# oxidecomputer/ingot

Measured on AMD Instinct MI355X. Metric: Mpkt/s device-resident L2/L3/L4 parse, 64–1500 B frames; % HBM roofline, higher is better.
Workload: dtype u8; 1 GPU; C2: 1,048,576 x 64 B Eth/IPv4/UDP per GPU, 64-B slots, UdpParser; frames_per_gpu=1048576, frames_total=1048576, chain=UdpParser, record_bytes=16, streams=2, arena_copies_rotated=8, record_buffers_rotated=8, timing_mode=launches

## Files before the change

### ingot_amd/csrc/ring.hip

```cpp
#include "walk.h"

namespace ingot_gpu {
namespace {

template <uint32_t NCH, uint32_t DEPTH, int CHAIN, int MODE, uint32_t POL = 0>
__global__ __launch_bounds__(BLOCK) void k_parse_pipe(ParseArgs a) {
    constexpr uint32_t WIN = NCH * 16u;
    const uint32_t pol = POL ? POL : a.policy;
    constexpr uint32_t WAVE_DW = WAVE * NCH * 4u;
    constexpr uint32_t IMG_DW = WAVES * WAVE_DW + 16u;
    __shared__ __attribute__((aligned(16))) uint32_t s_img[DEPTH * IMG_DW];
    const uint32_t lane = threadIdx.x & (WAVE - 1u);
    const uint32_t wave = threadIdx.x / WAVE;
    uint32_t* img0 = s_img + wave * WAVE_DW;
    const uint64_t ntiles = (a.n + WAVE - 1u) / WAVE;
    const uint32_t take = a.stride < WIN ? a.stride : WIN;

    auto stage = [&](uint64_t tt, uint32_t* img) {
#pragma unroll
        for (uint32_t k = 0; k < NCH; ++k) {
            const uint32_t q = k * WAVE + lane;
            const uint32_t pp = q / NCH;
            const uint32_t c = (q - pp * NCH) ^ swz<NCH>(pp);
            uint64_t slot = tt * WAVE + pp;
            if (slot >= a.n) slot = a.n - 1u;
            stage16p(a.arena + slot * a.stride + 16u * c, img + k * WAVE * 4u, pol);
        }
    };
    auto parse = [&](uint64_t tt, const uint32_t* img) {
        const uint64_t i = tt * WAVE + lane;
        Frame<NCH> fr{(const lds_u32*)img, lane, 0u, take, a.stride, a.arena + i * a.stride};
        Rec r;
        walk<CHAIN, false>(fr, r, nullptr, nullptr);
        if (i < a.n) {
            if constexpr (MODE == OUT_REC8) store_rec(static_cast<uint2*>(a.out) + i, pack8(r), pol);
            else store_rec(static_cast<uint4*>(a.out) + i, pack(r), pol);
        }
    };

    uint32_t bid = blockIdx.x;
    if ((a.xcd_remap & 1u) && gridDim.x % 8u == 0u)
        bid = (bid % 8u) * (gridDim.x / 8u) + bid / 8u;
    const uint64_t gw = (uint64_t)bid * WAVES + wave;
    const uint64_t nw = (uint64_t)gridDim.x * WAVES;
    uint64_t t, step, tend;
    if ((a.xcd_remap & 4u) && gridDim.x % 8u == 0u) {
        const uint64_t x = blockIdx.x % 8u;
        const uint64_t nwx = (uint64_t)(gridDim.x / 8u) * WAVES;
        const uint64_t region = (ntiles + 7u) / 8u;
        t = x * region + (uint64_t)(blockIdx.x / 8u) * WAVES + wave;
        tend = (x + 1u) * region < ntiles ? (x + 1u) * region : ntiles;
        step = nwx;
    } else if (a.xcd_remap & 2u) {
        const uint64_t J = (ntiles + nw - 1u) / nw;
        t = gw * J;
        tend = t + J < ntiles ? t + J : ntiles;
        step = 1u;
    } else {
        t = gw;
        tend = ntiles;
        step = nw;
    }
    if (t >= tend) return;
    if constexpr (DEPTH == 1) {
        stage(t, img0);
        asm volatile("s_waitcnt vmcnt(0)" ::: "memory");
        for (;;) {
            const uint64_t i = t * WAVE + lane;
            Frame<NCH> fr{(const lds_u32*)img0, lane, 0u, take, a.stride, a.arena + i * a.stride};
            Rec r;
            walk<CHAIN, false>(fr, r, nullptr, nullptr);
            asm volatile("s_waitcnt lgkmcnt(0)" ::: "memory");
            const uint64_t tn = t + step;
            const bool more = tn < tend;
            if (more) stage(tn, img0);
            if (i < a.n) {
                if constexpr (MODE == OUT_REC8) store_rec(static_cast<uint2*>(a.out) + i, pack8(r), pol);
                else store_rec(static_cast<uint4*>(a.out) + i, pack(r), pol);
            }
            if (!more) break;
            t = tn;
            asm volatile("s_waitcnt vmcnt(1)" ::: "memory");
        }
        return;
    }
#pragma unroll
    for (uint32_t d = 0; d + 1u < DEPTH; ++d)
        if (t + d * step < tend) stage(t + d * step, img0 + d * IMG_DW);
    for (uint32_t j = 0;; ++j) {
        const uint64_t tn = t + (DEPTH - 1u) * step;
        if (tn < tend) {
            stage(tn, img0 + ((j + DEPTH - 1u) % DEPTH) * IMG_DW);
            if (j + 1u >= DEPTH)
                asm volatile("s_waitcnt vmcnt(%0)" ::"n"((DEPTH - 1u) * (NCH + 1u)) : "memory");
            else
                asm volatile("s_waitcnt vmcnt(%0)" ::"n"((DEPTH - 1u) * NCH) : "memory");
        } else {
            asm volatile("s_waitcnt vmcnt(0)" ::: "memory");
        }
        parse(t, img0 + (j % DEPTH) * IMG_DW);
        t += step;
        if (t >= tend) break;
    }
}

__device__ __forceinline__ uint32_t load_system_u32(const uint32_t* p) {
    uint32_t v;
    asm volatile("global_load_dword %0, %1, off sc0 sc1\n\ts_waitcnt vmcnt(0)"
                 : "=v"(v)
                 : "v"(p)
                 : "memory");
    return (uint32_t)__builtin_amdgcn_readfirstlane((int)v);
}

template <uint32_t NCH, uint32_t DEPTH, int CHAIN, int MODE>
__global__ __launch_bounds__(BLOCK) void k_parse_ring(RingArgs a) {
    constexpr uint32_t WIN = NCH * 16u;
    constexpr uint32_t WAVE_DW = WAVE * NCH * 4u;
    constexpr uint32_t IMG_DW = WAVES * WAVE_DW + 16u;
    __shared__ __attribute__((aligned(16))) uint32_t s_img[DEPTH * IMG_DW];
    const uint32_t lane = threadIdx.x & (WAVE - 1u);
    const uint32_t wave = (uint32_t)__builtin_amdgcn_readfirstlane((int)(threadIdx.x / WAVE));
    uint32_t* img0 = s_img + wave * WAVE_DW;
    const uint32_t tpb = a.tiles_per_batch;
    const uint32_t G = a.groups;
    const uint32_t grp = (blockIdx.x / 8u) % G;
    const uint32_t gblk = (blockIdx.x / (8u * G)) * 8u + blockIdx.x % 8u;
    const uint32_t W = (gridDim.x / G) * WAVES;
    const uint32_t nbg = (a.nbatches - grp + G - 1u) / G;
    const uint32_t total = tpb * nbg;
    const uint32_t g0 = gblk * WAVES + wave;
    if (g0 >= total) return;
    const uint32_t J = (total - g0 + W - 1u) / W;
    uint64_t n = a.n;
    uint32_t stride = a.stride, policy = a.policy, nb = a.nbatches;
    asm volatile("" : "+s"(n), "+s"(stride), "+s"(policy), "+s"(nb));
    const uint32_t take = stride < WIN ? stride : WIN;
    uint32_t avail = a.published;
    bool live = true;

    auto ready = [&](uint32_t b) -> bool {
        if (b < avail) return true;
        if (!a.doorbell) return false;
        const uint64_t t0 = wall_clock64();
        uint32_t naps = 1;
        for (;;) {
            const uint32_t v = load_system_u32(a.doorbell);
            if (v >= a.db_first + b) {
                const uint32_t pub = v - a.db_first + 1u;
                avail = pub < a.nbatches ? pub : a.nbatches;
                __builtin_amdgcn_fence(__ATOMIC_ACQUIRE, "");
                return true;
            }
            if (wall_clock64() - t0 > a.timeout_ticks) {
                if (a.status && lane == 0) atomicOr(a.status, 1u);
                return false;
            }
            for (uint32_t z = 0; z < naps; ++z) __builtin_amdgcn_s_sleep(32);
            naps = naps < 8u ? 2u * naps : 8u;
        }
    };
    struct Cur {
        uint32_t b, t;
        const uint8_t* arena;
        void* out;
    };
    auto setb = [&](Cur& c) {
        if (c.b < nb) {
            c.arena = a.b[c.b].arena;
            c.out = a.b[c.b].out;
            asm volatile("" : "+s"(c.arena), "+s"(c.out));
        }
    };
    auto adv = [&](Cur& c) {
        c.t += W;
        if (c.t >= tpb) {
            do {
                c.t -= tpb;
                c.b += G;
            } while (c.t >= tpb);
            setb(c);
        }
    };
    Cur sc{grp + (g0 / tpb) * G, g0 % tpb, nullptr, nullptr};
    setb(sc);
    Cur pc = sc;
    auto stage = [&](const Cur& c, uint32_t* img) {
#pragma unroll
        for (uint32_t k = 0; k < NCH; ++k) {
            const uint32_t q = k * WAVE + lane;
            const uint32_t pp = q / NCH;
            const uint32_t ch = (q - pp * NCH) ^ swz<NCH>(pp);
            uint64_t slot = (uint64_t)c.t * WAVE + pp;
            if (slot >= n) slot = n - 1u;
            stage16p(c.arena + slot * stride + 16u * ch, img + k * WAVE * 4u, policy);
        }
    };
    auto parse = [&](const Cur& c, const uint32_t* img) {
        const uint64_t i = (uint64_t)c.t * WAVE + lane;
        Frame<NCH> fr{(const lds_u32*)img, lane, 0u, take, stride, c.arena + i * stride};
        Rec r;
        walk<CHAIN, false>(fr, r, nullptr, nullptr);
        if (i < n) {
            if constexpr (MODE == OUT_REC8)
                store_rec(static_cast<uint2*>(c.out) + i, pack8(r), policy);
            else
                store_rec(static_cast<uint4*>(c.out) + i, pack(r), policy);
        }
    };
    auto issue = [&](uint32_t& js) -> bool {
        if (!live || js >= J) return false;
        if (!ready(sc.b)) {
            live = false;
            return false;
        }
        stage(sc, img0 + (js % DEPTH) * IMG_DW);
        ++js;
        adv(sc);
        return true;
    };

    uint32_t js = 0;
#pragma unroll
    for (uint32_t d = 0; d + 1u < DEPTH; ++d) issue(js);
    for (uint32_t j = 0; j < js; ++j) {
        if (issue(js) && js - j == DEPTH) {
            if (j + 1u >= DEPTH)
                asm volatile("s_waitcnt vmcnt(%0)" ::"n"((DEPTH - 1u) * (NCH + 1u)) : "memory");
            else
                asm volatile("s_waitcnt vmcnt(%0)" ::"n"((DEPTH - 1u) * NCH) : "memory");
        } else {
            asm volatile("s_waitcnt vmcnt(0)" ::: "memory");
        }
        parse(pc, img0 + (j % DEPTH) * IMG_DW);
        adv(pc);
    }
}

template <uint32_t NCH, uint32_t DEPTH, int CHAIN>
__global__ __launch_bounds__(BLOCK) void k_modify_pipe(ModifyArgs m) {
    const ParseArgs& a = m.p;
    constexpr uint32_t WIN = NCH * 16u;
    constexpr uint32_t WAVE_DW = WAVE * NCH * 4u;
    constexpr uint32_t IMG_DW = WAVES * WAVE_DW + 16u;
    __shared__ __attribute__((aligned(16))) uint32_t s_img[DEPTH * IMG_DW];
    const uint32_t lane = threadIdx.x & (WAVE - 1u);
    const uint32_t wave = threadIdx.x / WAVE;
    uint32_t* img0 = s_img + wave * WAVE_DW;
    const uint64_t ntiles = (a.n + WAVE - 1u) / WAVE;
    const uint64_t step = (uint64_t)gridDim.x * WAVES;
    const bool nt_ld = a.policy & 1u;
    uint8_t* arena = const_cast<uint8_t*>(a.arena);
    const uint32_t unit_ch = m.wb / 16u;

    auto stage = [&](uint64_t tt, uint32_t* img) {
#pragma unroll
        for (uint32_t k = 0; k < NCH; ++k) {
            const uint32_t q = k * WAVE + lane;
            const uint32_t pp = q / NCH;
            const uint32_t c = (q - pp * NCH) ^ swz<NCH>(pp);
            uint64_t slot = tt * WAVE + pp;
            if (slot >= a.n) slot = a.n - 1u;
            stage16(a.arena + slot * a.stride + 16u * c, img + k * WAVE * 4u, nt_ld);
        }
    };
    auto modify = [&](uint64_t tt, uint32_t* img) {
        const uint64_t i = tt * WAVE + lane;
        const bool valid = i < a.n;
        uint8_t* frame = arena + (valid ? i : 0) * a.stride;
        Frame<NCH> fr{(const lds_u32*)img, lane, 0u, WIN, a.stride, frame};
        Rec r;
        walk<CHAIN, false>(fr, r, nullptr, nullptr);
        uint32_t dirty = 0;
        if (valid && r.status == INGOT_OK) {
            for (uint32_t k = 0; k < m.n_edits; ++k) {
                const Edit& e = m.e[k];
                uint32_t h;
                if (!header_at<CHAIN>(r, e.layer, e.kind, e.index, h)) continue;
                uint64_t w = fr.be(h + e.byte0, e.nbytes);
                const uint32_t fm = e.bits >= 32 ? 0xffffffffu : ((1u << e.bits) - 1u);
                const uint32_t cur = (uint32_t)(w >> e.rshift) & fm;
                uint32_t v;
                switch (e.op) {
                case INGOT_OP_ADD: v = cur + e.value; break;
                case INGOT_OP_SUB: v = cur - e.value; break;
                case INGOT_OP_AND: v = cur & e.value; break;
                case INGOT_OP_OR: v = cur | e.value; break;
                case INGOT_OP_XOR: v = cur ^ e.value; break;
                default: v = e.value; break;
                }
                w = (w & ~((uint64_t)fm << e.rshift)) | ((uint64_t)(v & fm) << e.rshift);
                for (uint32_t b = 0; b < e.nbytes; ++b) {
                    const uint32_t at = h + e.byte0 + b;
                    const uint8_t x = (uint8_t)(w >> (8u * (e.nbytes - 1u - b)));
                    if (at < WIN) {
                        fr.put_staged(at, x);
                        const uint32_t c0 = (at >> 4) & ~(unit_ch - 1u);
                        dirty |= ((1u << unit_ch) - 1u) << c0;
                    } else {
                        frame[at] = x;
                    }
                }
            }
        }
        if (valid && a.out) store_rec(static_cast<uint4*>(a.out) + i, pack(r), a.policy);
        __builtin_amdgcn_fence(__ATOMIC_RELEASE, "wavefront");
        __builtin_amdgcn_wave_barrier();
        __builtin_amdgcn_fence(__ATOMIC_ACQUIRE, "wavefront");
#pragma unroll
        for (uint32_t k = 0; k < NCH; ++k) {
            const uint32_t q = k * WAVE + lane;
            const uint32_t pp = q / NCH;
            const uint32_t c = (q - pp * NCH) ^ swz<NCH>(pp);
            const uint32_t d = (uint32_t)__shfl((int)dirty, (int)pp);
            if ((d >> c) & 1u) {
                const uint32_t* src = img + q * 4u;
                const uint4 v = make_uint4(src[0], src[1], src[2], src[3]);
                store_rec(reinterpret_cast<uint4*>(arena + (tt * WAVE + pp) * a.stride + 16u * c),
                          v, a.policy);
            }
        }
    };

    uint32_t bid = blockIdx.x;
    if ((a.xcd_remap & 1u) && gridDim.x % 8u == 0u)
        bid = (bid % 8u) * (gridDim.x / 8u) + bid / 8u;
    uint64_t t = (uint64_t)bid * WAVES + wave;
    if (t >= ntiles) return;
#pragma unroll
    for (uint32_t d = 0; d + 1u < DEPTH; ++d)
        if (t + d * step < ntiles) stage(t + d * step, img0 + d * IMG_DW);
    for (uint32_t j = 0;; ++j) {
        const uint64_t tn = t + (DEPTH - 1u) * step;
        if (tn < ntiles) {
            stage(tn, img0 + ((j + DEPTH - 1u) % DEPTH) * IMG_DW);
            asm volatile("s_waitcnt vmcnt(%0)" ::"n"((DEPTH - 1u) * NCH) : "memory");
        } else {
            asm volatile("s_waitcnt vmcnt(0)" ::: "memory");
        }
        modify(t, img0 + (j % DEPTH) * IMG_DW);
        asm volatile("s_waitcnt lgkmcnt(0)" ::: "memory");
        t += step;
        if (t >= ntiles) break;
    }
}

template <uint32_t DEPTH>
hipError_t launch_modify_pipe(const ModifyArgs& a, int chain, uint32_t grid, hipStream_t s) {
    switch (chain) {
    case INGOT_CHAIN_UDP_PARSER:
        hipLaunchKernelGGL((k_modify_pipe<4, DEPTH, INGOT_CHAIN_UDP_PARSER>), dim3(grid),
                           dim3(BLOCK), 0, s, a);
        break;
    case INGOT_CHAIN_GENERIC_ULP:
        hipLaunchKernelGGL((k_modify_pipe<4, DEPTH, INGOT_CHAIN_GENERIC_ULP>), dim3(grid),
                           dim3(BLOCK), 0, s, a);
        break;
    case INGOT_CHAIN_VLAN_ULP:
        hipLaunchKernelGGL((k_modify_pipe<4, DEPTH, INGOT_CHAIN_VLAN_ULP>), dim3(grid),
                           dim3(BLOCK), 0, s, a);
        break;
    default:
        return hipErrorInvalidValue;
    }
    return hipGetLastError();
}

template <uint32_t NCH, uint32_t DEPTH, int MODE, uint32_t POL = 0>
hipError_t launch_pipe(const ParseArgs& a, int chain, uint32_t grid, hipStream_t s) {
    switch (chain) {
    case INGOT_CHAIN_UDP_PARSER:
        hipLaunchKernelGGL((k_parse_pipe<NCH, DEPTH, INGOT_CHAIN_UDP_PARSER, MODE, POL>),
                           dim3(grid), dim3(BLOCK), 0, s, a);
        break;
    case INGOT_CHAIN_GENERIC_ULP:
        hipLaunchKernelGGL((k_parse_pipe<NCH, DEPTH, INGOT_CHAIN_GENERIC_ULP, MODE, POL>),
                           dim3(grid), dim3(BLOCK), 0, s, a);
        break;
    case INGOT_CHAIN_VLAN_ULP:
        hipLaunchKernelGGL((k_parse_pipe<NCH, DEPTH, INGOT_CHAIN_VLAN_ULP, MODE, POL>),
                           dim3(grid), dim3(BLOCK), 0, s, a);
        break;
    default:
        return hipErrorInvalidValue;
    }
    return hipGetLastError();
}

}

constexpr uint32_t kModifyRingWb = 64;
constexpr uint32_t kModifyRingPolicy = 3;

hipError_t launch_slot_ring(const ParseArgs& args, int chain, int mode, const Tuning& t,
                            hipStream_t s) {
    ParseArgs a = args;
    a.xcd_remap = t.xcd_remap == 0   ? 1u
                  : t.xcd_remap == 4 ? 0u
                  : t.xcd_remap == 5 ? 4u
                                     : (uint32_t)t.xcd_remap;
    const uint64_t tiles = (a.n + WAVE - 1) / WAVE;
    uint64_t blocks;
    if (t.pipeline > 1) {
        const uint64_t waves = (tiles + (uint64_t)t.pipeline - 1) / (uint64_t)t.pipeline;
        blocks = (waves + WAVES - 1) / WAVES;
    } else {
        const uint64_t cap = (t.ring_grid ? (uint64_t)t.ring_grid : 2ull) * t.cus;
        blocks = (tiles + WAVES - 1) / WAVES;
        if (blocks > cap) blocks = cap;
    }
    const uint32_t pg = (uint32_t)(blocks ? blocks : 1);
    if (t.pipe_depth == 0) {
        if (mode == OUT_REC16 && a.policy == 11u) return launch_pipe<4, 1, OUT_REC16, 11u>(a, chain, pg, s);
        if (mode == OUT_REC8 && a.policy == 3u) return launch_pipe<4, 1, OUT_REC8, 3u>(a, chain, pg, s);
        return mode == OUT_REC8 ? launch_pipe<4, 1, OUT_REC8>(a, chain, pg, s)
                                : launch_pipe<4, 1, OUT_REC16>(a, chain, pg, s);
    }
    if (t.pipe_depth == 3)
        return mode == OUT_REC8 ? launch_pipe<4, 3, OUT_REC8>(a, chain, pg, s)
                                : launch_pipe<4, 3, OUT_REC16>(a, chain, pg, s);
    if (t.pipe_depth == 4)
        return mode == OUT_REC8 ? launch_pipe<4, 4, OUT_REC8>(a, chain, pg, s)
                                : launch_pipe<4, 4, OUT_REC16>(a, chain, pg, s);
    if (mode == OUT_REC16 && a.policy == 11u) return launch_pipe<4, 2, OUT_REC16, 11u>(a, chain, pg, s);
    if (mode == OUT_REC8 && a.policy == 3u) return launch_pipe<4, 2, OUT_REC8, 3u>(a, chain, pg, s);
    return mode == OUT_REC8 ? launch_pipe<4, 2, OUT_REC8>(a, chain, pg, s)
                            : launch_pipe<4, 2, OUT_REC16>(a, chain, pg, s);
}

hipError_t launch_modify_ring(const ModifyArgs& args, int chain, const Tuning& t,
                              hipStream_t s) {
    ModifyArgs a = args;
    a.p.xcd_remap = t.xcd_remap == 0 ? 1u : t.xcd_remap == 4 ? 0u : ((uint32_t)t.xcd_remap & 1u);
    a.wb = t.writeback ? (uint32_t)t.writeback : kModifyRingWb;
    a.p.policy = t.cache_policy ? (uint32_t)t.cache_policy & 0x3bu : kModifyRingPolicy;
    const uint64_t tiles = (a.p.n + WAVE - 1) / WAVE;
    uint64_t blocks;
    if (t.pipeline > 1) {
        const uint64_t waves = (tiles + (uint64_t)t.pipeline - 1) / (uint64_t)t.pipeline;
        blocks = (waves + WAVES - 1) / WAVES;
    } else {
        const uint64_t cap = 2ull * t.cus;
        blocks = (tiles + WAVES - 1) / WAVES;
        if (blocks > cap) blocks = cap;
    }
    const uint32_t pg = (uint32_t)(blocks ? blocks : 1);
    return t.pipe_depth == 3 ? launch_modify_pipe<3>(a, chain, pg, s)
                             : launch_modify_pipe<2>(a, chain, pg, s);
}

template <uint32_t DEPTH, int MODE>
hipError_t launch_ring_chain(const RingArgs& a, int chain, uint32_t grid, hipStream_t s) {
    switch (chain) {
    case INGOT_CHAIN_UDP_PARSER:
        hipLaunchKernelGGL((k_parse_ring<4, DEPTH, INGOT_CHAIN_UDP_PARSER, MODE>), dim3(grid),
                           dim3(BLOCK), 0, s, a);
        break;
    case INGOT_CHAIN_GENERIC_ULP:
        hipLaunchKernelGGL((k_parse_ring<4, DEPTH, INGOT_CHAIN_GENERIC_ULP, MODE>), dim3(grid),
                           dim3(BLOCK), 0, s, a);
        break;
    case INGOT_CHAIN_VLAN_ULP:
        hipLaunchKernelGGL((k_parse_ring<4, DEPTH, INGOT_CHAIN_VLAN_ULP, MODE>), dim3(grid),
                           dim3(BLOCK), 0, s, a);
        break;
    default:
        return hipErrorInvalidValue;
    }
    return hipGetLastError();
}

hipError_t launch_ring(const RingArgs& args, int chain, int mode, const Tuning& t,
                       hipStream_t s) {
    RingArgs a = args;
    if (a.nbatches == 0 || a.n == 0) return hipSuccess;
    if (t.cache_policy == 0) a.policy = mode == OUT_REC16 ? 11u : 3u;
    else a.policy = (uint32_t)t.cache_policy & 0x1fbu;
    const uint64_t total = (uint64_t)a.tiles_per_batch * a.nbatches;
    const uint64_t bpc = t.ring_grid ? (uint64_t)t.ring_grid : 2ull;
    uint64_t blocks = (total + WAVES - 1) / WAVES;
    if (blocks > bpc * t.cus) blocks = bpc * t.cus;
    const uint32_t g = (uint32_t)(blocks ? blocks : 1);
    a.groups = t.ring_groups > 1 ? (uint32_t)t.ring_groups : 1u;
    if (g % (8u * a.groups) != 0 || a.groups > a.nbatches) a.groups = 1;
    const bool r8 = mode == OUT_REC8;
    switch (t.pipe_depth) {
    case 3: return r8 ? launch_ring_chain<3, OUT_REC8>(a, chain, g, s)
                      : launch_ring_chain<3, OUT_REC16>(a, chain, g, s);
    case 4: return r8 ? launch_ring_chain<4, OUT_REC8>(a, chain, g, s)
                      : launch_ring_chain<4, OUT_REC16>(a, chain, g, s);
    default: return r8 ? launch_ring_chain<2, OUT_REC8>(a, chain, g, s)
                       : launch_ring_chain<2, OUT_REC16>(a, chain, g, s);
    }
}

}
```

Measured before the change: 91160 Mpkt/s.

## Scalarize tile addressing and specialize 64-byte stride staging with immediate offsets

Reworks the pipelined parse kernel so tile base pointers live in scalar registers (readfirstlane on loop bounds and wave index) and lanes use precomputed 32-bit offsets instead of recomputing 64-bit per-lane slot addresses and clamps every tile. Adds a 64-byte-stride specialization that issues the four global_load_lds ops with immediate offsets, and stores records via scalar-base plus voffset asm stores. Tail clamping is moved to a single tail-tile branch. This aims to cut VALU address arithmetic in a memory-bound loop, in exchange for more code paths and inline asm store variants.

```diff
diff --git a/ingot_amd/csrc/ring.hip b/ingot_amd/csrc/ring.hip
--- a/ingot_amd/csrc/ring.hip
+++ b/ingot_amd/csrc/ring.hip
@@ -2,6 +2,55 @@
 
 namespace ingot_gpu {
 namespace {
+
+__device__ __forceinline__ uint64_t uniform64(uint64_t v) {
+    uint32_t lo = (uint32_t)__builtin_amdgcn_readfirstlane((int)(uint32_t)v);
+    uint32_t hi = (uint32_t)__builtin_amdgcn_readfirstlane((int)(uint32_t)(v >> 32));
+    asm volatile("" : "+s"(lo), "+s"(hi));
+    return ((uint64_t)hi << 32) | lo;
+}
+
+template <int OFF>
+__device__ __forceinline__ void stage16p_at(const uint8_t* src, uint32_t* dst, uint32_t pol) {
+#define INGOT_LD(bits) __builtin_amdgcn_global_load_lds((const void*)src, (lds_void*)dst, 16, OFF, bits)
+    switch ((pol >> 6) & 7u) {
+    case 1: INGOT_LD(16); return;
+    case 2: INGOT_LD(18); return;
+    case 3: INGOT_LD(17); return;
+    case 4: INGOT_LD(19); return;
+    case 5: INGOT_LD(1); return;
+    case 6: INGOT_LD(3); return;
+    default:
+        if (pol & 1u) INGOT_LD(2);
+        else INGOT_LD(0);
+    }
+#undef INGOT_LD
+}
+
+#define INGOT_ST(op, bits) asm volatile(op " %0, %1, %2 " bits "\n\ts_nop 1" ::"v"(voff), "v"(x), "s"(base) : "memory")
+#define INGOT_ST_SWITCH(op)                                    \
+    switch ((pol >> 3) & 7u) {                                 \
+    case 1: INGOT_ST(op, "sc1"); return;                       \
+    case 2: INGOT_ST(op, "sc1 nt"); return;                    \
+    case 3: INGOT_ST(op, "sc0 sc1"); return;                   \
+    case 4: INGOT_ST(op, "sc0 sc1 nt"); return;                \
+    case 5: INGOT_ST(op, "sc0"); return;                       \
+    default: if (pol & 2u) { INGOT_ST(op, "nt"); return; }     \
+    }
+__device__ __forceinline__ void store_rec_at(uint8_t* base, uint32_t voff, const uint4& v,
+                                             uint32_t pol) {
+    const u32x4 x{v.x, v.y, v.z, v.w};
+    INGOT_ST_SWITCH("global_store_dwordx4")
+    st_global(reinterpret_cast<uint4*>(base + voff), v);
+}
+__device__ __forceinline__ void store_rec_at(uint8_t* base, uint32_t voff, const uint2& v,
+                                             uint32_t pol) {
+    const u32x2 x{v.x, v.y};
+    INGOT_ST_SWITCH("global_store_dwordx2")
+    st_global(reinterpret_cast<uint2*>(base + voff), v);
+}
+#undef INGOT_ST_SWITCH
+#undef INGOT_ST
 
 template <uint32_t NCH, uint32_t DEPTH, int CHAIN, int MODE, uint32_t POL = 0>
 __global__ __launch_bounds__(BLOCK) void k_parse_pipe(ParseArgs a) {
@@ -10,33 +59,13 @@
     constexpr uint32_t WAVE_DW = WAVE * NCH * 4u;
     constexpr uint32_t IMG_DW = WAVES * WAVE_DW + 16u;
     __shared__ __attribute__((aligned(16))) uint32_t s_img[DEPTH * IMG_DW];
+    constexpr uint32_t REC_B = MODE == OUT_REC8 ? 8u : 16u;
     const uint32_t lane = threadIdx.x & (WAVE - 1u);
-    const uint32_t wave = threadIdx.x / WAVE;
+    const uint32_t wave = (uint32_t)__builtin_amdgcn_readfirstlane((int)(threadIdx.x / WAVE));
     uint32_t* img0 = s_img + wave * WAVE_DW;
     const uint64_t ntiles = (a.n + WAVE - 1u) / WAVE;
-    const uint32_t take = a.stride < WIN ? a.stride : WIN;
-
-    auto stage = [&](uint64_t tt, uint32_t* img) {
-#pragma unroll
-        for (uint32_t k = 0; k < NCH; ++k) {
-            const uint32_t q = k * WAVE + lane;
-            const uint32_t pp = q / NCH;
-            const uint32_t c = (q - pp * NCH) ^ swz<NCH>(pp);
-            uint64_t slot = tt * WAVE + pp;
-            if (slot >= a.n) slot = a.n - 1u;
-            stage16p(a.arena + slot * a.stride + 16u * c, img + k * WAVE * 4u, pol);
-        }
-    };
-    auto parse = [&](uint64_t tt, const uint32_t* img) {
-        const uint64_t i = tt * WAVE + lane;
-        Frame<NCH> fr{(const lds_u32*)img, lane, 0u, take, a.stride, a.arena + i * a.stride};
-        Rec r;
-        walk<CHAIN, false>(fr, r, nullptr, nullptr);
-        if (i < a.n) {
-            if constexpr (MODE == OUT_REC8) store_rec(static_cast<uint2*>(a.out) + i, pack8(r), pol);
-            else store_rec(static_cast<uint4*>(a.out) + i, pack(r), pol);
-        }
-    };
+    const uint64_t ttail = a.n % WAVE ? ntiles - 1u : ~0ull;
+    const uint32_t tail_last = (uint32_t)((a.n - 1u) % WAVE);
 
     uint32_t bid = blockIdx.x;
     if ((a.xcd_remap & 1u) && gridDim.x % 8u == 0u)
@@ -61,47 +90,127 @@
         tend = ntiles;
         step = nw;
     }
+    t = uniform64(t);
+    step = uniform64(step);
+    tend = uniform64(tend);
     if (t >= tend) return;
-    if constexpr (DEPTH == 1) {
-        stage(t, img0);
-        asm volatile("s_waitcnt vmcnt(0)" ::: "memory");
-        for (;;) {
-            const uint64_t i = t * WAVE + lane;
-            Frame<NCH> fr{(const lds_u32*)img0, lane, 0u, take, a.stride, a.arena + i * a.stride};
+    auto run = [&](auto s64) {
+        constexpr bool S64 = decltype(s64)::value;
+        static_assert(!S64 || NCH == 4, "the immediate-offset form is NCH == 4's");
+        const uint32_t stride = S64 ? 64u : a.stride;
+        const uint32_t take = stride < WIN ? stride : WIN;
+        uint32_t voff[NCH];
+#pragma unroll
+        for (uint32_t k = 0; k < NCH; ++k) {
+            const uint32_t q = k * WAVE + lane;
+            const uint32_t pp = q / NCH;
+            voff[k] = pp * stride + 16u * ((q - pp * NCH) ^ swz<NCH>(pp));
+        }
+        const uint32_t frame_off = lane * stride;
+        const uint32_t rec_off = lane * REC_B;
+        const uint64_t tile_b = (uint64_t)WAVE * stride;
+        const uint64_t dsrc = step * tile_b;
+        const uint64_t dout = step * (WAVE * REC_B);
+
+        auto stage = [&](uint64_t tt, const uint8_t* src, uint32_t* img) {
+            if (tt == ttail) {
+                uint32_t l = lane;
+                asm volatile("" : "+v"(l));
+#pragma unroll
+                for (uint32_t k = 0; k < NCH; ++k) {
+                    const uint32_t q = k * WAVE + l;
+                    const uint32_t pp = q / NCH;
+                    const uint32_t c = (q - pp * NCH) ^ swz<NCH>(pp);
+                    const uint32_t slot = pp < tail_last ? pp : tail_last;
+                    stage16p(src + (slot * stride + 16u * c), img + k * WAVE * 4u, pol);
+                }
+            } else if constexpr (S64) {
+                uint32_t vo = voff[0];
+                asm volatile("" : "+v"(vo));
+                stage16p_at<0>(src + vo, img, pol);
+                stage16p_at<1024>(src + vo, img, pol);
+                stage16p_at<2048>(src + vo, img, pol);
+                stage16p_at<3072>(src + vo, img, pol);
+            } else {
+#pragma unroll
+                for (uint32_t k = 0; k < NCH; ++k) {
+                    uint32_t vo = voff[k];
+                    asm volatile("" : "+v"(vo));
+                    stage16p(src + vo, img + k * WAVE * 4u, pol);
+                }
+            }
+        };
+        auto frame = [&](uint64_t tt, const uint8_t* src, const uint32_t* img) {
+            const uint8_t* g = nullptr;
+            if constexpr (!S64)
+                g = src + (tt == ttail && lane > tail_last ? tail_last * stride : frame_off);
+            return Frame<NCH>{(const lds_u32*)img, lane, 0u, take, stride, g};
+        };
+        auto emit = [&](uint64_t tt, uint8_t* dst, const Rec& r) {
+            if (tt == ttail && lane > tail_last) return;
+            if constexpr (MODE == OUT_REC8) store_rec_at(dst, rec_off, pack8(r), pol);
+            else store_rec_at(dst, rec_off, pack(r), pol);
+        };
+
+        const uint8_t* src = a.arena + t * tile_b;
+        uint8_t* dst = static_cast<uint8_t*>(a.out) + t * (WAVE * REC_B);
+        if constexpr (DEPTH == 1) {
+            stage(t, src, img0);
+            asm volatile("s_waitcnt vmcnt(0)" ::: "memory");
+            for (;;) {
+                Frame<NCH> fr = frame(t, src, img0);
+                Rec r;
+                walk<CHAIN, false>(fr, r, nullptr, nullptr);
+                asm volatile("s_waitcnt lgkmcnt(0)" ::: "memory");
+                const uint64_t tn = t + step;
+                const bool more = tn < tend;
+                if (more) stage(tn, src + dsrc, img0);
+                emit(t, dst, r);
+                if (!more) break;
+                t = tn;
+                src += dsrc;
+                dst += dout;
+                asm volatile("s_waitcnt vmcnt(1)" ::: "memory");
+            }
+            return;
+        }
+        uint64_t ts = t;
+        const uint8_t* ssrc = src;
+#pragma unroll
+        for (uint32_t d = 0; d + 1u < DEPTH; ++d) {
+            if (ts < tend) stage(ts, ssrc, img0 + d * IMG_DW);
+            ts += step;
+            ssrc += dsrc;
+        }
+        for (uint32_t j = 0;; ++j) {
+            if (ts < tend) {
+                stage(ts, ssrc, img0 + ((j + DEPTH - 1u) % DEPTH) * IMG_DW);
+                if (j + 1u >= DEPTH)
+                    asm volatile("s_waitcnt vmcnt(%0)" ::"n"((DEPTH - 1u) * (NCH + 1u)) : "memory");
+                else
+                    asm volatile("s_waitcnt vmcnt(%0)" ::"n"((DEPTH - 1u) * NCH) : "memory");
+            } else {
+                asm volatile("s_waitcnt vmcnt(0)" ::: "memory");
+            }
+            ts += step;
+            ssrc += dsrc;
+            Frame<NCH> fr = frame(t, src, img0 + (j % DEPTH) * IMG_DW);
             Rec r;
             walk<CHAIN, false>(fr, r, nullptr, nullptr);
-            asm volatile("s_waitcnt lgkmcnt(0)" ::: "memory");
-            const uint64_t tn = t + step;
-            const bool more = tn < tend;
-            if (more) stage(tn, img0);
-            if (i < a.n) {
-                if constexpr (MODE == OUT_REC8) store_rec(static_cast<uint2*>(a.out) + i, pack8(r), pol);
-                else store_rec(static_cast<uint4*>(a.out) + i, pack(r), pol);
-            }
-            if (!more) break;
-            t = tn;
-            asm volatile("s_waitcnt vmcnt(1)" ::: "memory");
-        }
-        return;
-    }
-#pragma unroll
-    for (uint32_t d = 0; d + 1u < DEPTH; ++d)
-        if (t + d * step < tend) stage(t + d * step, img0 + d * IMG_DW);
-    for (uint32_t j = 0;; ++j) {
-        const uint64_t tn = t + (DEPTH - 1u) * step;
-        if (tn < tend) {
-            stage(tn, img0 + ((j + DEPTH - 1u) % DEPTH) * IMG_DW);
-            if (j + 1u >= DEPTH)
-                asm volatile("s_waitcnt vmcnt(%0)" ::"n"((DEPTH - 1u) * (NCH + 1u)) : "memory");
-            else
-                asm volatile("s_waitcnt vmcnt(%0)" ::"n"((DEPTH - 1u) * NCH) : "memory");
-        } else {
-            asm volatile("s_waitcnt vmcnt(0)" ::: "memory");
-        }
-        parse(t, img0 + (j % DEPTH) * IMG_DW);
-        t += step;
-        if (t >= tend) break;
-    }
+            emit(t, dst, r);
+            t += step;
+            if (t >= tend) break;
+            src += dsrc;
+            dst += dout;
+        }
+    };
+    if constexpr (NCH == 4) {
+        if (a.stride == 64u) {
+            run(std::true_type{});
+            return;
+        }
+    }
+    run(std::false_type{});
 }
 
 __device__ __forceinline__ uint32_t load_system_u32(const uint32_t* p) {
```

Result: faster. 92930 Mpkt/s (median of 6 runs) (+1.9%).
